# jialeli1/From-Voxel-to-Point

Measured on AMD Instinct MI355X. Metric: point clouds/sec fwd+bwd (FV2P, KITTI shape) at 1/2/4/8 MI355X, higher is better.
Workload: dtype f32

## Files before the change

### from-voxel-to-point_amd/fv2p_harness/fv2p_model.py

```python
import math
import os
from functools import partial

import numpy as np
import torch
import torch.nn as nn
import torch.nn.functional as F

from pcdet.ops.iou3d_nms import iou3d_nms_cuda, iou3d_nms_utils
from pcdet.ops.pointnet2.pointnet2_batch import pointnet2_modules as pn2_batch_modules
from pcdet.ops.pointnet2.pointnet2_batch import fused as pn2_fused
from pcdet.ops.pointnet2.pointnet2_batch import pointnet2_utils as pn2_batch
from pcdet.ops.pointnet2.pointnet2_stack import pointnet2_utils as pn2_stack
from pcdet.ops.roiaware_pool3d import roiaware_pool3d_utils
from pcdet.ops.roipoint_pool3d import roipoint_pool3d_utils
from pcdet.models.backbones_3d.pfe import bev_grid_pooling

import fv2p_native as _nat

from .backbone import VoxelResBackBone8x, bn_act

TWO_PI = 2.0 * math.pi


class FV2PConfig:
    point_cloud_range = (0.0, -40.0, -3.0, 70.4, 40.0, 1.0)
    voxel_size = (0.05, 0.05, 0.1)
    grid_size = (1408, 1600, 40)
    max_points_per_voxel, max_voxels = 5, 16000
    num_point_features = 4
    bev_layers, bev_strides, bev_filters = (5, 5), (1, 2), (128, 256)
    bev_up_strides, bev_up_filters = (1, 2), (256, 256)
    anchor_rotations = (0.0, 1.57)
    anchor_classes = (((3.9, 1.6, 1.56), -1.78, 0.6, 0.45), ((0.8, 0.6, 1.73), -0.6, 0.5, 0.35), ((1.76, 0.6, 1.73), -0.6, 0.5, 0.35))
    dir_offset, dir_limit_offset, num_dir_bins = 0.78539, 0.0, 2
    rpn_w = dict(cls=1.0, loc=2.0, dir=0.2)
    num_keypoints = 16384
    decode_levels = (("x_conv4", 8, 128, 256), ("x_conv3", 4, 64, 192), ("x_conv2", 2, 32, 160), ("x_conv1", 1, 16, 128))
    init_source, init_stride, init_channels = "x_conv4", 8, 128
    decoder_out = 128
    point_cls_fc, gt_extra_width, point_cls_weight = (64, 64), (0.2, 0.2, 0.2), 4.0
    nms_pre, nms_post, nms_thresh = 9000, 512, 0.8
    roi_per_image, fg_ratio = 128, 0.5
    cls_fg, cls_bg, cls_bg_lo, reg_fg, hard_bg_ratio = 0.75, 0.25, 0.1, 0.55, 0.8
    pool_extra_width, num_sampled_points, depth_normalizer = (3.2, 3.2, 3.2), 512, 70.0
    xyz_up, grid_size_roi = (128, 128), 6
    sa_radii, sa_nsamples, sa_mlps = (0.8, 1.6), (16, 32), ((64, 64), (64, 64))
    bev_pool_in, bev_pool_out = 512, 128
    interact_filters, cge_up, cge_interact, fuse_filters = (256, 256), (64, 64), (128,), (256,)
    cls_fc, reg_fc, dp_ratio = (256, 256), (256, 256), 0.3
    grad_norm_clip = 10.0
    key_stream = True
    point_branch_stream = True
    dense_branch_stream = False


class FV2PWaymoConfig(FV2PConfig):
    point_cloud_range = (-75.2, -75.2, -2.0, 75.2, 75.2, 4.0)
    voxel_size = (0.1, 0.1, 0.15)
    grid_size = (1504, 1504, 40)
    max_voxels = 80000
    num_point_features = 5
    bev_layers = (3, 3)
    anchor_classes = (((4.7, 2.1, 1.7), 0.0, 0.55, 0.4),)


KERNEL_GLUE = True
LINEAR_CHUNK_ROWS = 1024
FULL_NMS = False
_SIDE_STREAMS = {}
_CONSTS = {}
_CORNER_SIGNS = ((1, 1, -1), (1, -1, -1), (-1, -1, -1), (-1, 1, -1), (1, 1, 1), (1, -1, 1), (-1, -1, 1), (-1, 1, 1))


def dconst(like, values, dtype=torch.float32):
    key = (like.device, dtype, values)
    t = _CONSTS.get(key)
    if t is None:
        t = _CONSTS[key] = torch.tensor(values, dtype=dtype, device=like.device)
    return t


def side_stream(role, device):
    key = (role, torch.device(device).index)
    if key not in _SIDE_STREAMS:
        high = role in os.environ.get("FV2P_STREAM_PRIO", "dense").split(",")
        _SIDE_STREAMS[key] = torch.cuda.Stream(device=device, priority=-1 if high else 0)
    return _SIDE_STREAMS[key]


def limit_period(val, offset, period):
    return val - torch.floor(val / period + offset) * period


def rotate_z(points, angle):
    c, s = torch.cos(angle), torch.sin(angle)
    x, y = points[..., 0], points[..., 1]
    xr = x * c[:, None] - y * s[:, None]
    yr = x * s[:, None] + y * c[:, None]
# ... 2 lines not shown

def residual_encode(boxes, anchors):
    a_sz = anchors[..., 3:6].clamp_min(1e-5)
    b_sz = boxes[..., 3:6].clamp_min(1e-5)
    diag = torch.sqrt(a_sz[..., 0:1] ** 2 + a_sz[..., 1:2] ** 2)
    xy = (boxes[..., 0:2] - anchors[..., 0:2]) / diag
    z = (boxes[..., 2:3] - anchors[..., 2:3]) / a_sz[..., 2:3]
    return torch.cat((xy, z, torch.log(b_sz / a_sz), boxes[..., 6:7] - anchors[..., 6:7]), dim=-1)


def residual_decode(enc, anchors):
    a_sz = anchors[..., 3:6]
    diag = torch.sqrt(a_sz[..., 0:1] ** 2 + a_sz[..., 1:2] ** 2)
    xy = enc[..., 0:2] * diag + anchors[..., 0:2]
    z = enc[..., 2:3] * a_sz[..., 2:3] + anchors[..., 2:3]
    return torch.cat((xy, z, torch.exp(enc[..., 3:6]) * a_sz, enc[..., 6:7] + anchors[..., 6:7]), dim=-1)


def sigmoid_focal(logits, onehot, weights, alpha=0.25, gamma=2.0):
    p = torch.sigmoid(logits)
    alpha_w = onehot * alpha + (1 - onehot) * (1 - alpha)
    pt = onehot * (1.0 - p) + (1.0 - onehot) * p
    bce = logits.clamp(min=0) - logits * onehot + torch.log1p(torch.exp(-logits.abs()))
    return alpha_w * pt.pow(gamma) * bce * weights.unsqueeze(-1)


def smooth_l1(diff, beta):
    n = diff.abs()
    return torch.where(n < beta, 0.5 * n * n / beta, n - 0.5 * beta)


def box_corners(boxes):
    t = dconst(boxes, _CORNER_SIGNS, boxes.dtype) / 2
    c = boxes[:, None, 3:6] * t[None]
    return rotate_z(c, boxes[:, 6]) + boxes[:, None, 0:3]


def corner_loss_lidar(pred, gt):
    pc, gc = box_corners(pred), box_corners(gt)
    gflip = box_corners(torch.cat((gt[:, :6], gt[:, 6:7] + math.pi), dim=1))
    dist = torch.minimum((pc - gc).norm(dim=2), (pc - gflip).norm(dim=2))
    return smooth_l1(dist, 1.0).mean(dim=1)


def nearest_bev_boxes(b):
    rot = limit_period(b[..., 6], 0.5, math.pi).abs()
    swap = (rot >= math.pi / 4).unsqueeze(-1)
    dims = torch.where(swap, b[..., 3:5].flip(-1), b[..., 3:5])
    return torch.cat((b[..., 0:2] - dims / 2, b[..., 0:2] + dims / 2), dim=-1)


def mlp1d(cin, widths, out=None, conv=False, bn_kw=None, dropout_after_first=None):
    mk = (lambda a, b, bias: nn.Conv1d(a, b, 1, bias=bias)) if conv else (lambda a, b, bias: nn.Linear(a, b, bias=bias))
    layers = []
    for i, w in enumerate(widths):
        layers += [mk(cin, w, False), nn.BatchNorm1d(w, **(bn_kw or {})), nn.ReLU()]
        if dropout_after_first is not None and i == 0:
            layers.append(nn.Dropout(dropout_after_first))
        cin = w
    if out is not None:
        layers.append(mk(cin, out, True))
    return nn.Sequential(*layers)


def run_rows(seq, x):
    mods = list(seq)
    i = 0
    while i < len(mods):
        m = mods[i]
        if isinstance(m, nn.BatchNorm1d) and x.dim() == 2:
            relu = mods[i + 1] if i + 1 < len(mods) and isinstance(mods[i + 1], nn.ReLU) else None
            x = bn_act(m, x, relu)
            i += 1 + (relu is not None)
        elif (KERNEL_GLUE and type(m) is nn.Linear and x.dim() == 2 and x.is_cuda and x.shape[0] >= 4 * LINEAR_CHUNK_ROWS
              and x.shape[0] % LINEAR_CHUNK_ROWS == 0 and "forward" not in m.__dict__):
            x = rows_linear(x.reshape(-1, LINEAR_CHUNK_ROWS, x.shape[1]), m.weight, m.bias).reshape(x.shape[0], -1)
            i += 1
        else:
            x = m(x)
            i += 1
    return x


class BEVBackbone(nn.Module):

    def __init__(self, cfg, cin):
        super().__init__()
        bn = partial(nn.BatchNorm2d, eps=1e-3, momentum=0.01)
        self.blocks, self.deblocks = nn.ModuleList(), nn.ModuleList()
        for n, s, f, us, uf in zip(cfg.bev_layers, cfg.bev_strides, cfg.bev_filters, cfg.bev_up_strides, cfg.bev_up_filters):
            seq = [nn.ZeroPad2d(1), nn.Conv2d(cin, f, 3, stride=s, padding=0, bias=False), bn(f), nn.ReLU()]
            for _ in range(n):
                seq += [nn.Conv2d(f, f, 3, padding=1, bias=False), bn(f), nn.ReLU()]
            self.blocks.append(nn.Sequential(*seq))
            self.deblocks.append(nn.Sequential(nn.ConvTranspose2d(f, uf, us, stride=us, bias=False), bn(uf), nn.ReLU()))
            cin = f
        self.num_bev_features = sum(cfg.bev_up_filters)

    def forward(self, x):
        ups = []
        for blk, de in zip(self.blocks, self.deblocks):
            x = self._block(blk, x)
            ups.append(de(x))
        return torch.cat(ups, dim=1)

    @staticmethod
    def _block(blk, x):
        mods = list(blk)
        if (KERNEL_GLUE and len(mods) >= 2 and isinstance(mods[0], nn.ZeroPad2d) and type(mods[1]) is nn.Conv2d and "forward" not in mods[1].__dict__
                and tuple(mods[0].padding) == (1, 1, 1, 1) and tuple(mods[1].padding) == (0, 0) and mods[1].padding_mode == "zeros"):
            c = mods[1]
            x = F.conv2d(x, c.weight, c.bias, c.stride, (1, 1), c.dilation, c.groups)
            mods = mods[2:]
        for m in mods:
            x = m(x)
        return x


class AnchorLossFn(torch.autograd.Function):

    @staticmethod
    def forward(ctx, cls, box, dirs, labels, reg_t, anchor_rot, cfg):
        b, a = labels.shape
        out = cls.new_empty(4)
        dcls, dbox, ddirs = torch.empty_like(cls), torch.empty_like(box), torch.empty_like(dirs)
        with _nat.device_guard(cls.device):
            ws = _nat.workspace(int(_nat.lib().fv2p_anchor_loss_ws_bytes(b, a)), cls.device)
            _nat.call("fv2p_anchor_loss", cls, box, dirs, labels, reg_t, anchor_rot, b, a, 0.25, 1.0 / 9.0, float(cfg.dir_offset),
                      float(cfg.rpn_w["cls"]), float(cfg.rpn_w["loc"]), float(cfg.rpn_w["dir"]), out, dcls, dbox, ddirs, ws, ws.numel(), _nat.stream())
        ctx.save_for_backward(dcls, dbox, ddirs)
        return out[0]

    @staticmethod
    def backward(ctx, g):
        dcls, dbox, ddirs = ctx.saved_tensors
        return dcls * g, dbox * g, ddirs * g, None, None, None, None


class AnchorHead(nn.Module):

    def __init__(self, cfg, cin):
        super().__init__()
        self.cfg = cfg
        nr, nc = len(cfg.anchor_rotations), len(cfg.anchor_classes)
        na = nr * nc
        self.conv_cls = nn.Conv2d(cin, na, 1)
        self.conv_box = nn.Conv2d(cin, na * 7, 1)
        self.conv_dir_cls = nn.Conv2d(cin, na * cfg.num_dir_bins, 1)
        nn.init.constant_(self.conv_cls.bias, -math.log((1 - 0.01) / 0.01))
        nn.init.normal_(self.conv_box.weight, mean=0, std=0.001)
        r = cfg.point_cloud_range
        w, h = cfg.grid_size[0] // 8, cfg.grid_size[1] // 8
        xs = torch.arange(r[0], r[3] + 1e-5, step=(r[3] - r[0]) / (w - 1), dtype=torch.float32)
        ys = torch.arange(r[1], r[4] + 1e-5, step=(r[4] - r[1]) / (h - 1), dtype=torch.float32)
        a = torch.zeros(h, w, nc, nr, 7)
        a[..., 0] = xs.view(1, w, 1, 1)
        a[..., 1] = ys.view(h, 1, 1, 1)
        for c, (size, bottom, _, _) in enumerate(cfg.anchor_classes):
            a[:, :, c, :, 3:6] = torch.tensor(size)
            a[:, :, c, :, 2] = bottom
        a[..., 6] = torch.tensor(cfg.anchor_rotations).view(1, 1, 1, nr)
        a[..., 2] += a[..., 5] / 2
        self.register_buffer("anchors", a.view(-1, 7), persistent=False)
        self.register_buffer("anchor_rot", a.view(-1, 7)[:, 6].contiguous(), persistent=False)
        for c in range(nc):
            ac = a[:, :, c].reshape(-1, 7).contiguous()
            self.register_buffer(f"anchors_c{c}", ac, persistent=False)
            self.register_buffer(f"anchor_bev_c{c}", nearest_bev_boxes(ac), persistent=False)

    @torch.no_grad()
    def assign(self, gt):
        cfg = self.cfg
        nc, nr, b = len(cfg.anchor_classes), len(cfg.anchor_rotations), gt.shape[0]
        labels, regs = [], []
        for c, (_, _, matched, unmatched) in enumerate(cfg.anchor_classes):
            gt_c = gt if nc == 1 else torch.where((gt[..., 7:8] == c + 1), gt, torch.zeros_like(gt))
            one = self.assign_one_kernel if (gt.is_cuda and gt.shape[-1] >= 8 and KERNEL_GLUE) else self.assign_one_tensor_ops
            lab, reg = one(gt_c, getattr(self, f"anchors_c{c}"), getattr(self, f"anchor_bev_c{c}"), matched, unmatched)
            labels.append(lab.view(b, -1, 1, nr))
            regs.append(reg.view(b, -1, 1, nr, 7))
        if nc == 1:
            return labels[0].view(b, -1), regs[0].view(b, -1, 7)
        return torch.cat(labels, dim=2).reshape(b, -1), torch.cat(regs, dim=2).reshape(b, -1, 7)

    def assign_tensor_ops(self, gt):
        cfg = self.cfg
        nc, nr, b = len(cfg.anchor_classes), len(cfg.anchor_rotations), gt.shape[0]
        labels, regs = [], []
        for c, (_, _, matched, unmatched) in enumerate(cfg.anchor_classes):
            gt_c = gt if nc == 1 else torch.where((gt[..., 7:8] == c + 1), gt, torch.zeros_like(gt))
            lab, reg = self.assign_one_tensor_ops(gt_c, getattr(self, f"anchors_c{c}"), getattr(self, f"anchor_bev_c{c}"), matched, unmatched)
            labels.append(lab.view(b, -1, 1, nr))
            regs.append(reg.view(b, -1, 1, nr, 7))
        return torch.cat(labels, dim=2).reshape(b, -1), torch.cat(regs, dim=2).reshape(b, -1, 7)

    @staticmethod
    @torch.no_grad()
    def assign_one_kernel(gt, anchors, anchor_bev, matched, unmatched):
        b, g, a = gt.shape[0], gt.shape[1], anchors.shape[0]
# ... 574 lines not shown
```

### from-voxel-to-point_amd/fv2p_harness/mgaf_model.py

```python
from functools import partial

import math

import torch
import torch.nn as nn
import torch.nn.functional as F

from pcdet.ops.DeformableConvolutionV2PyTorch.modules.mdeformable_conv_block import MdeformConvBlock
from pcdet.ops.DeformableConvolutionV2PyTorch.modules.modulated_deform_conv import ModulatedDeformConv

from pcdet.ops.iou3d_nms import iou3d_nms_utils

from .backbone import VoxelResBackBone8x
from .fv2p_model import box_corners, sigmoid_focal


class MGAFConfig:
    grid_size = (1408, 1600, 40)
    num_point_features = 4
    layer_nums, layer_strides, num_filters = (5, 5, 5), (1, 2, 2), (128, 256, 256)
    upsample_strides, num_upsample_filters = (1, 2, 4), (256, 256, 256)
    shared_fc = (256,)
    head_deformable_groups = 4
    heads = (("hm", 3), ("offset", 2), ("height", 1), ("dim", 3), ("rot", 24), ("segm", 1), ("iouscore", 1))
    head_conv = 128
    point_cloud_range = (0.0, -40.0, -3.0, 70.4, 40.0, 1.0)
    voxel_size = (0.05, 0.05, 0.1)
    feature_map_stride, gaussian_minoverlap, gaussian_minradius, max_objs = 8, 0.01, 2, 50
    num_iouscore_training_samples = 24
    loss_weights = dict(hm=1.0, offset=1.0, height=1.0, dim=1.0, rot=1.0, segm=1.0, corner=1.0, iouscore=1.0)
    rot_bins, iou_fg_thresh, iou_bg_thresh = 12, 0.75, 0.25


class DCNBEVBackbone(nn.Module):
    def __init__(self, cfg, cin):
        super().__init__()
        bn = partial(nn.BatchNorm2d, eps=1e-3, momentum=0.01)
        self.blocks, self.deblocks = nn.ModuleList(), nn.ModuleList()
        for n, s, f, us, uf in zip(cfg.layer_nums, cfg.layer_strides, cfg.num_filters, cfg.upsample_strides, cfg.num_upsample_filters):
            seq = [nn.ZeroPad2d(1), nn.Conv2d(cin, f, 3, stride=s, padding=0, bias=False), bn(f), nn.ReLU()]
            for _ in range(n):
                seq += [nn.Conv2d(f, f, 3, padding=1, bias=False), bn(f), nn.ReLU()]
            self.blocks.append(nn.Sequential(*seq))
            self.deblocks.append(nn.Sequential(MdeformConvBlock(f, f, deformable_groups=1), bn(f), nn.ReLU(),
                                               nn.ConvTranspose2d(f, uf, us, stride=us, bias=False), bn(uf), nn.ReLU()))
            cin = f
        self.num_bev_features = sum(cfg.num_upsample_filters)

    def forward(self, x):
        ups = []
        from .fv2p_model import BEVBackbone
        for blk, de in zip(self.blocks, self.deblocks):
            x = BEVBackbone._block(blk, x)
            ups.append(de(x))
        return torch.cat(ups, dim=1)


class FeatureAdaption(nn.Module):

    def __init__(self, channels, deformable_groups):
        super().__init__()
        self.conv_offset_mask = nn.Conv2d(channels, deformable_groups * 27, 3, padding=1, bias=True)
        self.conv_adaption = ModulatedDeformConv(channels, channels, stride=1, kernel_size=3, padding=1, deformable_groups=deformable_groups, bias=False)

    def forward(self, x):
        o1, o2, mask = torch.chunk(self.conv_offset_mask(x), 3, dim=1)
        return torch.relu(self.conv_adaption(x, torch.cat((o1, o2), dim=1), torch.sigmoid(mask)))


class CenterAFHead(nn.Module):
    def __init__(self, cfg, cin):
        super().__init__()
        layers, pre = [], cin
        for f in cfg.shared_fc:
            layers += [nn.Conv2d(pre, f, 3, padding=1, bias=False), nn.BatchNorm2d(f), nn.ReLU()]
            pre = f
        self.shared_conv_layer = nn.Sequential(*layers)
        self.feature_adapt = FeatureAdaption(pre, cfg.head_deformable_groups)
        self.heads = nn.ModuleDict({name: nn.Sequential(nn.Conv2d(pre, cfg.head_conv, 3, padding=1, bias=False),
                                                        nn.BatchNorm2d(cfg.head_conv, eps=1e-3, momentum=0.01), nn.ReLU(),
                                                        nn.Conv2d(cfg.head_conv, out, 1, bias=True)) for name, out in cfg.heads})

    def forward(self, x):
        x = self.feature_adapt(self.shared_conv_layer(x))
        segm = self.heads["segm"](x)
        att = x + torch.sigmoid(segm.detach()).expand_as(x) * x
        preds = {"segm": segm}
        for name, head in self.heads.items():
            if name != "segm":
                preds[name] = head(att)
        return preds


def gaussian_radius(h, w, min_overlap):
    b1 = h + w
    c1 = w * h * (1 - min_overlap) / (1 + min_overlap)
    r1 = (b1 - torch.sqrt(b1 ** 2 - 4 * c1)) / 2
    b2 = 2 * (h + w)
    c2 = (1 - min_overlap) * w * h
    r2 = (b2 - torch.sqrt(b2 ** 2 - 16 * c2)) / 8
    a3 = 4 * min_overlap
    b3 = -2 * min_overlap * (h + w)
    c3 = (min_overlap - 1) * w * h
    r3 = (b3 + torch.sqrt(b3 ** 2 - 4 * a3 * c3)) / (2 * a3)
    return torch.minimum(torch.minimum(r1, r2), r3)


@torch.no_grad()
def center_targets(gt, cfg, num_classes):
    dev, b, m = gt.device, gt.shape[0], gt.shape[1]
    k = cfg.max_objs
    lo = torch.tensor(cfg.point_cloud_range[:3], dtype=torch.float32, device=dev)
    hi = torch.tensor(cfg.point_cloud_range[3:], dtype=torch.float32, device=dev)
    vs = torch.tensor(cfg.voxel_size, dtype=torch.float64, device=dev)
    stride = cfg.feature_map_stride
    sy = int(round((cfg.point_cloud_range[4] - cfg.point_cloud_range[1]) / cfg.voxel_size[1] / stride))
    sx = int(round((cfg.point_cloud_range[3] - cfg.point_cloud_range[0]) / cfg.voxel_size[0] / stride))
    boxes = gt[:, :, :7]
    nonzero = boxes.sum(-1) != 0
    pos = torch.arange(m, device=dev)
    last = torch.where(nonzero, pos, torch.zeros_like(pos)).amax(1)
    kk = min(k, m)
    bx = boxes[:, :kk]
    live = (pos[:kk][None] <= last[:, None])
    cls = gt[:, :kk, 7].to(torch.int8).long() - 1
    dimx = bx[..., 3].double() / vs[0] / stride
    dimy = bx[..., 4].double() / vs[1] / stride
    ok = live & (dimx > 0) & (dimy > 0)
    radius = gaussian_radius(torch.ceil(dimx), torch.ceil(dimy), cfg.gaussian_minoverlap)
    radius = torch.where(ok, radius, torch.zeros_like(radius)).nan_to_num(0.0).clamp(min=0).long().clamp(min=cfg.gaussian_minradius)
    cx = (bx[..., 0] - lo[0]).double() / vs[0] / stride
    cy = (bx[..., 1] - lo[1]).double() / vs[1] / stride
    cxi, cyi = torch.round(cx).long(), torch.round(cy).long()
    ok = ok & (cxi >= 0) & (cxi < sx) & (cyi >= 0) & (cyi < sy)
    ys = torch.arange(sy, device=dev).view(1, 1, sy, 1)
    xs = torch.arange(sx, device=dev).view(1, 1, 1, sx)
    dy, dx = ys - cyi[..., None, None], xs - cxi[..., None, None]
    r = radius[..., None, None]
# ... 171 lines not shown
```

### from-voxel-to-point_amd/pcdet/ops/spconv/norm.py

```python
import os

import torch
from torch import nn
from torch.autograd import Function

import fv2p_native as _nat

_ENABLED = os.environ.get("FV2P_FUSED_BN", "1") != "0"


_WS_BYTES = {}


def _ws_bytes(c):
    b = _WS_BYTES.get(c)
    if b is None:
        b = _WS_BYTES[c] = _nat.call("fv2p_batchnorm_ws_bytes", 0, c)
    return b


class _BatchNormReLU(Function):
    @staticmethod
    def forward(ctx, x, weight, bias, bn, relu):
        n, c = x.shape
        dev = x.device
        batch_stats = bn.training or bn.running_mean is None
        y = torch.empty_like(x)
        with _nat.device_guard(dev):
            if batch_stats:
                stats = torch.empty((2, c), dtype=torch.float32, device=dev)
                mean, invstd = stats[0], stats[1]
                track = bn.training and bn.running_mean is not None
                ws = _nat.workspace(_ws_bytes(c), dev)
                _nat.call("fv2p_batchnorm_forward", x, n, c, float(bn.eps), -1.0 if bn.momentum is None else float(bn.momentum),
                          weight, bias, int(relu), bn.running_mean if track else None, bn.running_var if track else None,
                          bn.num_batches_tracked if track else None, mean, invstd, y, ws, ws.numel(), _nat.stream())
            else:
                mean = bn.running_mean
                invstd = torch.rsqrt(bn.running_var + bn.eps)
                _nat.call("fv2p_batchnorm_apply", x, n, c, mean, invstd, weight, bias, int(relu), y, _nat.stream())
        ctx.save_for_backward(x, mean, invstd, weight, bias)
        ctx.relu, ctx.batch_stats = bool(relu), bool(batch_stats)
        return y

    @staticmethod
    def backward(ctx, dy):
        x, mean, invstd, weight, bias = ctx.saved_tensors
        n, c = x.shape
        dev = x.device
        dy = dy.contiguous()
        dx = torch.empty_like(x)
        dpar = torch.empty((2, c), dtype=torch.float32, device=dev)
        dgamma, dbeta = dpar[0], dpar[1]
        with _nat.device_guard(dev):
            ws = _nat.workspace(_ws_bytes(c), dev)
            _nat.call("fv2p_batchnorm_backward", x, dy, n, c, mean, invstd, weight, bias, int(ctx.relu), int(ctx.batch_stats),
                      dx, dgamma, dbeta, ws, ws.numel(), _nat.stream())
        return (dx if ctx.needs_input_grad[0] else None, dgamma if (weight is not None and ctx.needs_input_grad[1]) else None,
                dbeta if (bias is not None and ctx.needs_input_grad[2]) else None, None, None)


def _plain(module):
    return not (module._forward_hooks or module._forward_pre_hooks or module._backward_hooks)


def fusable(bn, relu_module, x, channels):
    if not _ENABLED or type(bn) is not nn.BatchNorm1d or not _plain(bn):
        return False
    if relu_module is not None and (type(relu_module) is not nn.ReLU or not _plain(relu_module)):
        return False
    if not (torch.is_tensor(x) and x.is_cuda and x.dtype == torch.float32 and x.dim() == 2):
        return False
    if torch.is_autocast_enabled() or channels != bn.num_features:
        return False
    c = channels
    if c > 256 and c % 4 != 0 or c > 1024:
        return False
    if bn.weight is not None and (bn.weight.dtype != torch.float32 or not bn.weight.is_cuda):
        return False
    return True


def batch_norm_relu(bn, x, relu_module=None):
    if not (torch.is_tensor(x) and x.dim() == 2 and x.is_contiguous() and fusable(bn, relu_module, x, x.shape[1])):
        return None
    if x.shape[0] < 2:
        return None
    ext = _nat.torch_ext()
    if ext is not None:
        return ext.batch_norm_relu(x, bn.weight, bn.bias, bn.running_mean, bn.running_var, bn.num_batches_tracked, bn.training,
                                   -1.0 if bn.momentum is None else float(bn.momentum), float(bn.eps), relu_module is not None)
    return _BatchNormReLU.apply(x, bn.weight, bn.bias, bn, relu_module is not None)
```

### include/fv2p_ops.h

```cpp
#ifndef FV2P_OPS_H_
#define FV2P_OPS_H_

#include <stddef.h>
#include <stdint.h>

#ifdef __cplusplus
extern "C" {
#endif

#define FV2P_ABI_VERSION 1

#define FV2P_EINVAL      (-1)
#define FV2P_EWORKSPACE  (-2)
#define FV2P_EHIP        (-3)
#define FV2P_ELIMIT      (-4)

typedef void* fv2p_stream_t;

const char* fv2p_last_error(void);
int fv2p_abi_version(void);

size_t fv2p_scan_ws_bytes(int64_t n);
int fv2p_exclusive_scan_i32(const int* in, int* out, int64_t n, int* total, void* ws, size_t ws_bytes,
                            fv2p_stream_t stream);
// ... 267 lines not shown
                      int deformable_group, float* dx_nhwc, float* doffset, float* dmask, float* dwt, void* ws,
                      size_t ws_bytes, fv2p_stream_t stream);
int fv2p_dcn_forward_grouped(const float* x_nhwc, const float* wt_oc, const float* bias, const float* offset,
                             const float* mask, int batch, int height, int width, int c_in, int c_out, int h_out,
                             int w_out, int kh, int kw, int sh, int sw, int ph, int pw, int dh, int dw,
                             int deformable_group, int group, float* y_nhwc, fv2p_stream_t stream);
size_t fv2p_dcn_backward_grouped_ws_bytes(int batch, int height, int width, int h_out, int w_out, int c_in, int c_out, int kh,
                                          int kw, int deformable_group, int group);
int fv2p_dcn_backward_grouped(const float* x_nhwc, const float* wt, const float* offset, const float* mask,
                              const float* dy_nhwc, int batch, int height, int width, int c_in, int c_out, int h_out,
                              int w_out, int kh, int kw, int sh, int sw, int ph, int pw, int dh, int dw,
                              int deformable_group, int group, float* dx_nhwc, float* doffset, float* dmask, float* dwt,
                              void* ws, size_t ws_bytes, fv2p_stream_t stream);

int fv2p_transpose_batched(const float* in, int batch, int64_t rows, int64_t cols, float* out, fv2p_stream_t stream);

int fv2p_deform_psroi_pool_forward(const float* data, const float* rois, const float* trans, int batch, int channels,
                                   int height, int width, int num_rois, int no_trans, float spatial_scale,
                                   int output_dim, int group_size, int pooled_size, int part_size,
                                   int sample_per_part, float trans_std, int num_classes, float* out,
                                   float* top_count, fv2p_stream_t stream);
int fv2p_deform_psroi_pool_backward(const float* grad_out, const float* data, const float* rois, const float* trans,
                                    const float* top_count, int batch, int channels, int height, int width,
                                    int num_rois, int no_trans, float spatial_scale, int output_dim,
                                    int group_size, int pooled_size, int part_size, int sample_per_part,
                                    float trans_std, int num_classes, float* grad_data, float* grad_trans,
                                    fv2p_stream_t stream);
size_t fv2p_deform_psroi_pool_backward_ws_bytes(int num_rois, int output_dim, int pooled_size, int sample_per_part);
int fv2p_deform_psroi_pool_backward_gather(const float* grad_out, const float* data, const float* rois, const float* trans,
                                           const float* top_count, int batch, int channels, int height, int width,
                                           int num_rois, int no_trans, float spatial_scale, int output_dim,
                                           int group_size, int pooled_size, int part_size, int sample_per_part,
                                           float trans_std, int num_classes, float* grad_data, float* grad_trans,
                                           void* ws, size_t ws_bytes, fv2p_stream_t stream);

size_t fv2p_batchnorm_ws_bytes(int64_t n, int c);
int fv2p_batchnorm_forward(const float* x, int64_t n, int c, float eps, float momentum, const float* gamma,
                           const float* beta, int relu, float* running_mean, float* running_var,
                           int64_t* num_batches_tracked, float* mean, float* invstd, float* y, void* ws,
                           size_t ws_bytes, fv2p_stream_t stream);
int fv2p_batchnorm_forward_stats(const float* x, int64_t n, int c, float eps, float momentum, const float* gamma,
                                 const float* beta, int relu, float* running_mean, float* running_var,
                                 int64_t* num_batches_tracked, float* mean, float* invstd, float* y,
                                 const double* stats, double* zero_next, int64_t zero_count, fv2p_stream_t stream);
int fv2p_batchnorm_backward_stats(const float* x, const float* dy, int64_t n, int c, const float* mean,
                                  const float* invstd, const float* gamma, const float* beta, int relu,
                                  int batch_stats, float* dx, float* dgamma, float* dbeta, const double* stats,
                                  double* zero_next, int64_t zero_count, fv2p_stream_t stream);
int fv2p_batchnorm_apply_res(const float* x, int64_t n, int c, const float* mean, const float* invstd, const float* gamma,
                             const float* beta, int relu, const float* residual, float* y, fv2p_stream_t stream);
int fv2p_batchnorm_backward_fin(const float* x, const float* dy, int64_t n, int c, const float* mean, const float* invstd,
                                const float* gamma, const float* beta, int relu, const float* coef, float* dx,
                                fv2p_stream_t stream);
int fv2p_batchnorm_backward_res(const float* x, const float* out, const float* dout, int64_t n, int c, const float* mean,
                                const float* invstd, const float* gamma, const float* beta, int batch_stats, float* dx,
                                float* dz, float* dgamma, float* dbeta, void* ws, size_t ws_bytes, fv2p_stream_t stream);
size_t fv2p_batchnorm_one_ws_bytes(int c);
int fv2p_batchnorm_one_pays(int64_t n, int c, int backward);
int fv2p_batchnorm_forward_one(const float* x, int64_t n, int c, float eps, float momentum, const float* gamma, const float* beta,
                               int relu, float* running_mean, float* running_var, int64_t* num_batches_tracked, float* mean,
                               float* invstd, const float* residual, float* y, void* ws, size_t ws_bytes, unsigned* counters,
                               fv2p_stream_t stream);
int fv2p_batchnorm_backward_one(const float* x, const float* dy, int64_t n, int c, const float* mean, const float* invstd,
                                const float* gamma, const float* beta, int relu, int batch_stats, const float* mask_y, float* dx,
                                float* dz_out, float* dgamma, float* dbeta, void* ws, size_t ws_bytes, unsigned* counters,
                                fv2p_stream_t stream);
size_t fv2p_batchnorm_wide_ws_bytes(int c);
int fv2p_batchnorm_wide_counter_words(int c);
int fv2p_batchnorm_forward_wide(const float* x, int64_t n, int c, float eps, float momentum, const float* gamma, const float* beta,
                                int relu, float* running_mean, float* running_var, int64_t* num_batches_tracked, float* mean,
                                float* invstd, const float* residual, float* y, void* ws, size_t ws_bytes, unsigned* counters,
                                fv2p_stream_t stream);
int fv2p_batchnorm_backward_wide(const float* x, const float* dy, int64_t n, int c, const float* mean, const float* invstd,
                                 const float* gamma, const float* beta, int relu, int batch_stats, const float* mask_y, float* dx,
                                 float* dz_out, float* dgamma, float* dbeta, void* ws, size_t ws_bytes, unsigned* counters,
                                 fv2p_stream_t stream);
int fv2p_batchnorm_apply(const float* x, int64_t n, int c, const float* mean, const float* invstd,
                         const float* gamma, const float* beta, int relu, float* y, fv2p_stream_t stream);
int fv2p_batchnorm_backward(const float* x, const float* dy, int64_t n, int c, const float* mean,
                            const float* invstd, const float* gamma, const float* beta, int relu, int batch_stats,
                            float* dx, float* dgamma, float* dbeta, void* ws, size_t ws_bytes,
                            fv2p_stream_t stream);

#ifdef __cplusplus
}
#endif
#endif
```

Baseline: 104.5.

## Fuse BatchNorm2d+ReLU in BEV backbone and write deblock outputs into concat buffer

```diff
diff --git a/from-voxel-to-point_amd/csrc/batchnorm2d.hip b/from-voxel-to-point_amd/csrc/batchnorm2d.hip
--- /dev/null
+++ b/from-voxel-to-point_amd/csrc/batchnorm2d.hip
@@ -0,0 +1,328 @@
+#include "common.hpp"
+#include "bn_fold.hpp"
+
+namespace fv2p {
+
+struct Bn2dGeom {
+  int b, c, k;
+  long long plane;
+  long long chunk;
+};
+
+constexpr long long kBn2dChunk = 8192;
+constexpr int kBn2dMaxChunks = 64;
+constexpr int kBn2dSerialFold = 32;
+
+static void bn2d_geom(int b, int c, long long plane, Bn2dGeom* g) {
+  long long k = (plane + kBn2dChunk / 2) / kBn2dChunk;
+  if (k < 1) k = 1;
+  if (k > kBn2dMaxChunks) k = kBn2dMaxChunks;
+  long long chunk = ceil_div(ceil_div(plane, k), 4) * 4;
+  k = ceil_div(plane, chunk);
+  g->b = b; g->c = c; g->k = static_cast<int>(k); g->plane = plane; g->chunk = chunk;
+}
+
+__device__ __forceinline__ void bn2d_block(const Bn2dGeom& g, int* b, int* c, int* k) {
+  const unsigned id = blockIdx.x;
+  *k = static_cast<int>(id % g.k);
+  const unsigned pl = id / g.k;
+  *c = static_cast<int>(pl % g.c);
+  *b = static_cast<int>(pl / g.c);
+}
+
+__device__ __forceinline__ void bn2d_block_sum(double& a, double& b, double (*red)[4]) {
+#pragma unroll
+  for (int off = 32; off >= 1; off >>= 1) {
+    a += __shfl_down(a, off, 64);
+    b += __shfl_down(b, off, 64);
+  }
+  const int tid = threadIdx.x;
+  if ((tid & 63) == 0) { red[0][tid >> 6] = a; red[1][tid >> 6] = b; }
+  __syncthreads();
+  if (tid == 0) {
+    a = ((red[0][0] + red[0][1]) + red[0][2]) + red[0][3];
+    b = ((red[1][0] + red[1][1]) + red[1][2]) + red[1][3];
+  }
+}
+
+__device__ __forceinline__ void bn2d_fold(const double* __restrict__ p, int count, double (*red)[256], double* a_out, double* b_out) {
+  double a = 0.0, b = 0.0;
+  if (count <= kBn2dSerialFold) {
+    for (int q = 0; q < count; ++q) { a += p[2 * q]; b += p[2 * q + 1]; }
+  } else {
+    const int tid = threadIdx.x;
+    for (int q = tid; q < count; q += 256) { a += p[2 * q]; b += p[2 * q + 1]; }
+    red[0][tid] = a; red[1][tid] = b;
+    __syncthreads();
+    for (int s = 128; s >= 1; s >>= 1) {
+      if (tid < s) { red[0][tid] += red[0][tid + s]; red[1][tid] += red[1][tid + s]; }
+      __syncthreads();
+    }
+    a = red[0][0]; b = red[1][0];
+  }
+  *a_out = a; *b_out = b;
+}
+
+template <int V>
+struct Vec2d;
+template <>
+struct Vec2d<4> {
+  float v[4];
+  __device__ __forceinline__ void load(const float* p) { const float4 q = *reinterpret_cast<const float4*>(p); v[0] = q.x; v[1] = q.y; v[2] = q.z; v[3] = q.w; }
+  __device__ __forceinline__ void store(float* p) const { *reinterpret_cast<float4*>(p) = make_float4(v[0], v[1], v[2], v[3]); }
+};
+template <>
+struct Vec2d<1> {
+  float v[1];
+  __device__ __forceinline__ void load(const float* p) { v[0] = *p; }
+  __device__ __forceinline__ void store(float* p) const { *p = v[0]; }
+};
+
+template <int V, bool BWD>
+__global__ __launch_bounds__(256) void bn2d_reduce_k(const float* __restrict__ x, const float* __restrict__ dy, long long dy_bstride, int dy_coff,
+                                                     Bn2dGeom g, const float* __restrict__ mean, const float* __restrict__ invstd,
+                                                     const float* __restrict__ gamma, const float* __restrict__ beta, int relu,
+                                                     double* __restrict__ partial, long long* __restrict__ nbt, long long* __restrict__ nbt_copy) {
+  __shared__ double red[2][4];
+  int b, c, k;
+  bn2d_block(g, &b, &c, &k);
+  const int tid = threadIdx.x;
+  if (!BWD && nbt && blockIdx.x == 0 && tid == 0) {
+    const long long seen = *nbt;
+    *nbt_copy = seen;
+    *nbt = seen + 1;
+  }
+  const long long e0 = static_cast<long long>(k) * g.chunk;
+  const long long e1 = min(e0 + g.chunk, g.plane);
+  const float* xp = x + (static_cast<long long>(b) * g.c + c) * g.plane;
+  const float* gp = BWD ? dy + static_cast<long long>(b) * dy_bstride + static_cast<long long>(dy_coff + c) * g.plane : nullptr;
+  float m = 0.f, is = 0.f, ga = 1.f, be = 0.f;
+  if (BWD) { m = mean[c]; is = invstd[c]; ga = gamma ? gamma[c] : 1.f; be = beta ? beta[c] : 0.f; }
+  double s1 = 0.0, s2 = 0.0;
+  auto accumulate = [&](const Vec2d<V>& xv, const Vec2d<V>& gv) {
+#pragma unroll
+    for (int i = 0; i < V; ++i) {
+      if (!BWD) {
+        const double d = xv.v[i];
+        s1 += d; s2 += d * d;
+      } else {
+        const float xhat = (xv.v[i] - m) * is;
+        const float t = xhat * ga + be;
+        const float dz = (relu && !(t > 0.f)) ? 0.f : gv.v[i];
+        s1 += dz; s2 += static_cast<double>(dz) * xhat;
+      }
+    }
+  };
+  constexpr int U = 4;
+  constexpr long long step = 256 * V;
+  long long e = e0 + static_cast<long long>(tid) * V;
+  for (; e + (U - 1) * step < e1; e += U * step) {
+    Vec2d<V> xv[U], gv[U];
+#pragma unroll
+    for (int u = 0; u < U; ++u) {
+      xv[u].load(xp + e + u * step);
+      if (BWD) gv[u].load(gp + e + u * step);
+    }
+#pragma unroll
+    for (int u = 0; u < U; ++u) accumulate(xv[u], gv[u]);
+  }
+  for (; e < e1; e += step) {
+    Vec2d<V> xv, gv;
+    xv.load(xp + e);
+    if (BWD) gv.load(gp + e);
+    accumulate(xv, gv);
+  }
+  bn2d_block_sum(s1, s2, red);
+  if (tid == 0) {
+    double* p = partial + ((static_cast<long long>(c) * g.b + b) * g.k + k) * 2;
+    p[0] = s1; p[1] = s2;
+  }
+}
+
+template <int V>
+__global__ __launch_bounds__(256) void bn2d_apply_fwd_k(const float* __restrict__ x, Bn2dGeom g, const double* __restrict__ partial, BnFwdFin ff,
+                                                        const float* __restrict__ gamma, const float* __restrict__ beta, int relu,
+                                                        float* __restrict__ y, long long y_bstride, int y_coff) {
+  __shared__ double red[2][256];
+  __shared__ float sh[2];
+  int b, c, k;
+  bn2d_block(g, &b, &c, &k);
+  const int tid = threadIdx.x;
+  const int count = g.b * g.k;
+  double sa, sb;
+  bn2d_fold(partial + static_cast<long long>(c) * count * 2, count, red, &sa, &sb);
+  if (tid == 0) {
+    float mu_f, is_f;
+    bn_fwd_channel(sa, sb, static_cast<long long>(g.b) * g.plane, ff, c, b == 0 && k == 0, &mu_f, &is_f);
+    sh[0] = mu_f; sh[1] = is_f;
+  }
+  __syncthreads();
+  const float m = sh[0], is = sh[1];
+  const float ga = gamma ? gamma[c] : 1.f, be = beta ? beta[c] : 0.f;
+  const long long e0 = static_cast<long long>(k) * g.chunk;
+  const long long e1 = min(e0 + g.chunk, g.plane);
+  const float* xp = x + (static_cast<long long>(b) * g.c + c) * g.plane;
+  float* yp = y + static_cast<long long>(b) * y_bstride + static_cast<long long>(y_coff + c) * g.plane;
+  auto apply = [&](const Vec2d<V>& xv, Vec2d<V>& o) {
+#pragma unroll
+    for (int i = 0; i < V; ++i) {
+      const float xhat = (xv.v[i] - m) * is;
+      const float t = xhat * ga + be;
+      o.v[i] = (relu && t <= 0.f) ? 0.f : t;
+    }
+  };
+  constexpr int U = 4;
+  constexpr long long step = 256 * V;
+  long long e = e0 + static_cast<long long>(tid) * V;
+  for (; e + (U - 1) * step < e1; e += U * step) {
+    Vec2d<V> xv[U], o[U];
+#pragma unroll
+    for (int u = 0; u < U; ++u) xv[u].load(xp + e + u * step);
+#pragma unroll
+    for (int u = 0; u < U; ++u) { apply(xv[u], o[u]); o[u].store(yp + e + u * step); }
+  }
+  for (; e < e1; e += step) {
+    Vec2d<V> xv, o;
+    xv.load(xp + e);
+    apply(xv, o);
+    o.store(yp + e);
+  }
+}
+
+template <int V>
+__global__ __launch_bounds__(256) void bn2d_apply_bwd_k(const float* __restrict__ x, const float* __restrict__ dy, long long dy_bstride, int dy_coff,
+                                                        Bn2dGeom g, const double* __restrict__ partial, const float* __restrict__ mean,
+                                                        const float* __restrict__ invstd, const float* __restrict__ gamma,
+                                                        const float* __restrict__ beta, int relu, float* __restrict__ dx,
+                                                        float* __restrict__ dgamma, float* __restrict__ dbeta) {
+  __shared__ double red[2][256];
+  int b, c, k;
+  bn2d_block(g, &b, &c, &k);
+  const int tid = threadIdx.x;
+  const int count = g.b * g.k;
+  double sa, sb;
+  bn2d_fold(partial + static_cast<long long>(c) * count * 2, count, red, &sa, &sb);
+  if (tid == 0 && b == 0 && k == 0) {
+    dbeta[c] = static_cast<float>(sa);
+    dgamma[c] = static_cast<float>(sb);
+  }
+  const double n = static_cast<double>(g.b) * static_cast<double>(g.plane);
+  const float c1 = static_cast<float>(sa / n), c2 = static_cast<float>(sb / n);
+  const float m = mean[c], is = invstd[c];
+  const float ga = gamma ? gamma[c] : 1.f, be = beta ? beta[c] : 0.f;
+  const long long e0 = static_cast<long long>(k) * g.chunk;
+  const long long e1 = min(e0 + g.chunk, g.plane);
+  const long long xoff = (static_cast<long long>(b) * g.c + c) * g.plane;
+  const float* xp = x + xoff;
+  float* dxp = dx + xoff;
+  const float* gp = dy + static_cast<long long>(b) * dy_bstride + static_cast<long long>(dy_coff + c) * g.plane;
+  auto apply = [&](const Vec2d<V>& xv, const Vec2d<V>& gv, Vec2d<V>& o) {
+#pragma unroll
+    for (int i = 0; i < V; ++i) {
+      const float xhat = (xv.v[i] - m) * is;
+      const float t = xhat * ga + be;
+      const float dz = (relu && !(t > 0.f)) ? 0.f : gv.v[i];
+      o.v[i] = ga * is * (dz - c1 - xhat * c2);
+    }
+  };
+  constexpr int U = 4;
+  constexpr long long step = 256 * V;
+  long long e = e0 + static_cast<long long>(tid) * V;
+  for (; e + (U - 1) * step < e1; e += U * step) {
+    Vec2d<V> xv[U], gv[U], o[U];
+#pragma unroll
+    for (int u = 0; u < U; ++u) { xv[u].load(xp + e + u * step); gv[u].load(gp + e + u * step); }
+#pragma unroll
+    for (int u = 0; u < U; ++u) { apply(xv[u], gv[u], o[u]); o[u].store(dxp + e + u * step); }
+  }
+  for (; e < e1; e += step) {
+    Vec2d<V> xv, gv, o;
+    xv.load(xp + e);
+    gv.load(gp + e);
+    apply(xv, gv, o);
+    o.store(dxp + e);
+  }
+}
+
+static bool bn2d_aligned16(const void* p) { return (reinterpret_cast<uintptr_t>(p) & 15) == 0; }
+
+static int bn2d_check(const char* who, int b, int c, int64_t plane, int64_t bstride, int coff) {
+  FV2P_REQUIRE(b >= 1 && c >= 1 && plane >= 1, FV2P_EINVAL, "%s: b=%d c=%d plane=%lld", who, b, c, static_cast<long long>(plane));
+  FV2P_REQUIRE(static_cast<long long>(b) * plane >= 2, FV2P_EINVAL, "%s: one value per channel", who);
+  FV2P_REQUIRE(coff >= 0 && bstride >= static_cast<int64_t>(coff + c) * plane, FV2P_EINVAL, "%s: channels %d..%d do not fit a batch stride of %lld", who,
+               coff, coff + c, static_cast<long long>(bstride));
+  return 0;
+}
+
+}
+
+using namespace fv2p;
+
+extern "C" size_t fv2p_batchnorm2d_ws_bytes(int b, int c, int64_t plane) {
+  Bn2dGeom g;
+  bn2d_geom(b > 0 ? b : 1, c > 0 ? c : 1, plane > 0 ? plane : 1, &g);
+  Sizer s;
+  s.take<double>(static_cast<size_t>(g.c) * g.b * g.k * 2);
+  s.take<long long>(1);
+  return s.bytes();
+}
+
+extern "C" int fv2p_batchnorm2d_forward(const float* x, int b, int c, int64_t plane, float eps, float momentum, const float* gamma,
+                                        const float* beta, int relu, float* running_mean, float* running_var, int64_t* num_batches_tracked,
+                                        float* mean, float* invstd, float* y, int64_t y_batch_stride, int y_channel_offset, void* ws,
+                                        size_t ws_bytes, fv2p_stream_t stream_) {
+  hipStream_t stream = static_cast<hipStream_t>(stream_);
+  if (int rc = bn2d_check("batchnorm2d_forward", b, c, plane, y_batch_stride, y_channel_offset)) return rc;
+  FV2P_REQUIRE(x && y && mean && invstd && ws, FV2P_EINVAL, "batchnorm2d_forward: null pointer");
+  FV2P_REQUIRE((running_mean == nullptr) == (running_var == nullptr), FV2P_EINVAL, "batchnorm2d_forward: running_mean and running_var come together");
+  FV2P_REQUIRE(ws_bytes >= fv2p_batchnorm2d_ws_bytes(b, c, plane), FV2P_EWORKSPACE, "batchnorm2d_forward: workspace %lld < %lld",
+               static_cast<long long>(ws_bytes), static_cast<long long>(fv2p_batchnorm2d_ws_bytes(b, c, plane)));
+  Bn2dGeom g;
+  bn2d_geom(b, c, plane, &g);
+  const int64_t blocks = static_cast<int64_t>(b) * c * g.k;
+  FV2P_REQUIRE(blocks <= 0x7fffffff, FV2P_ELIMIT, "batchnorm2d_forward: %lld workgroups", static_cast<long long>(blocks));
+  Carver cv(ws, ws_bytes);
+  double* partial = cv.take<double>(static_cast<size_t>(g.c) * g.b * g.k * 2);
+  long long* nbt_copy = cv.take<long long>(1);
+  long long* nbt = (running_mean && num_batches_tracked) ? reinterpret_cast<long long*>(num_batches_tracked) : nullptr;
+  BnFwdFin ff{mean, invstd, running_mean, running_var, nbt ? nbt_copy : nullptr, momentum, eps};
+  const bool vec = (plane % 4 == 0) && bn2d_aligned16(x) && bn2d_aligned16(y) && (y_batch_stride % 4 == 0);
+  const dim3 grid(static_cast<unsigned>(blocks)), wg(256);
+  if (vec) {
+    hipLaunchKernelGGL((bn2d_reduce_k<4, false>), grid, wg, 0, stream, x, nullptr, 0ll, 0, g, nullptr, nullptr, nullptr, nullptr, 0, partial, nbt, nbt_copy);
+    hipLaunchKernelGGL((bn2d_apply_fwd_k<4>), grid, wg, 0, stream, x, g, partial, ff, gamma, beta, relu, y, static_cast<long long>(y_batch_stride), y_channel_offset);
+  } else {
+    hipLaunchKernelGGL((bn2d_reduce_k<1, false>), grid, wg, 0, stream, x, nullptr, 0ll, 0, g, nullptr, nullptr, nullptr, nullptr, 0, partial, nbt, nbt_copy);
+    hipLaunchKernelGGL((bn2d_apply_fwd_k<1>), grid, wg, 0, stream, x, g, partial, ff, gamma, beta, relu, y, static_cast<long long>(y_batch_stride), y_channel_offset);
+  }
+  FV2P_LAUNCH_CHECK();
+  return 0;
+}
+
+extern "C" int fv2p_batchnorm2d_backward(const float* x, const float* dy, int64_t dy_batch_stride, int dy_channel_offset, int b, int c,
+                                         int64_t plane, const float* mean, const float* invstd, const float* gamma, const float* beta,
+                                         int relu, float* dx, float* dgamma, float* dbeta, void* ws, size_t ws_bytes, fv2p_stream_t stream_) {
+  hipStream_t stream = static_cast<hipStream_t>(stream_);
+  if (int rc = bn2d_check("batchnorm2d_backward", b, c, plane, dy_batch_stride, dy_channel_offset)) return rc;
+  FV2P_REQUIRE(x && dy && mean && invstd && dx && dgamma && dbeta && ws, FV2P_EINVAL, "batchnorm2d_backward: null pointer");
+  FV2P_REQUIRE(ws_bytes >= fv2p_batchnorm2d_ws_bytes(b, c, plane), FV2P_EWORKSPACE, "batchnorm2d_backward: workspace %lld < %lld",
+               static_cast<long long>(ws_bytes), static_cast<long long>(fv2p_batchnorm2d_ws_bytes(b, c, plane)));
+  Bn2dGeom g;
+  bn2d_geom(b, c, plane, &g);
+  const int64_t blocks = static_cast<int64_t>(b) * c * g.k;
+  FV2P_REQUIRE(blocks <= 0x7fffffff, FV2P_ELIMIT, "batchnorm2d_backward: %lld workgroups", static_cast<long long>(blocks));
+  Carver cv(ws, ws_bytes);
+  double* partial = cv.take<double>(static_cast<size_t>(g.c) * g.b * g.k * 2);
+  const bool vec = (plane % 4 == 0) && bn2d_aligned16(x) && bn2d_aligned16(dy) && bn2d_aligned16(dx) && (dy_batch_stride % 4 == 0);
+  const dim3 grid(static_cast<unsigned>(blocks)), wg(256);
+  const long long gs = static_cast<long long>(dy_batch_stride);
+  if (vec) {
+    hipLaunchKernelGGL((bn2d_reduce_k<4, true>), grid, wg, 0, stream, x, dy, gs, dy_channel_offset, g, mean, invstd, gamma, beta, relu, partial, nullptr, nullptr);
+    hipLaunchKernelGGL((bn2d_apply_bwd_k<4>), grid, wg, 0, stream, x, dy, gs, dy_channel_offset, g, partial, mean, invstd, gamma, beta, relu, dx, dgamma, dbeta);
+  } else {
+    hipLaunchKernelGGL((bn2d_reduce_k<1, true>), grid, wg, 0, stream, x, dy, gs, dy_channel_offset, g, mean, invstd, gamma, beta, relu, partial, nullptr, nullptr);
+    hipLaunchKernelGGL((bn2d_apply_bwd_k<1>), grid, wg, 0, stream, x, dy, gs, dy_channel_offset, g, partial, mean, invstd, gamma, beta, relu, dx, dgamma, dbeta);
+  }
+  FV2P_LAUNCH_CHECK();
+  return 0;
+}
diff --git a/from-voxel-to-point_amd/fv2p_harness/fv2p_model.py b/from-voxel-to-point_amd/fv2p_harness/fv2p_model.py
--- a/from-voxel-to-point_amd/fv2p_harness/fv2p_model.py
+++ b/from-voxel-to-point_amd/fv2p_harness/fv2p_model.py
@@ -15,6 +15,7 @@
 from pcdet.ops.roiaware_pool3d import roiaware_pool3d_utils
 from pcdet.ops.roipoint_pool3d import roipoint_pool3d_utils
 from pcdet.models.backbones_3d.pfe import bev_grid_pooling
+from pcdet.ops.spconv.norm import batch_norm_relu_2d, batch_norm_relu_2d_cat
 
 import fv2p_native as _nat
 
@@ -183,6 +184,39 @@
     return x
 
 
+def dense_seq(mods, x):
+    i = 0
+    while i < len(mods):
+        m = mods[i]
+        if KERNEL_GLUE and type(m) is nn.BatchNorm2d:
+            relu = mods[i + 1] if i + 1 < len(mods) and type(mods[i + 1]) is nn.ReLU else None
+            y = batch_norm_relu_2d(m, x, relu)
+            if y is not None:
+                x = y
+                i += 1 + (relu is not None)
+                continue
+        x = m(x)
+        i += 1
+    return x
+
+
+def deblock_head(de, x):
+    mods = list(de)
+    if (KERNEL_GLUE and len(mods) >= 3 and type(mods[-2]) is nn.BatchNorm2d and type(mods[-1]) is nn.ReLU
+            and not (de._forward_hooks or de._forward_pre_hooks or de._backward_hooks)):
+        return mods[-2], dense_seq(mods[:-2], x), mods[-1]
+    return de(x)
+
+
+def cat_deblocks(ups):
+    if len(ups) > 1 and all(isinstance(u, tuple) for u in ups):
+        y = batch_norm_relu_2d_cat(ups)
+        if y is not None:
+            return y
+    ups = [dense_seq([u[0], u[2]], u[1]) if isinstance(u, tuple) else u for u in ups]
+    return torch.cat(ups, dim=1) if len(ups) > 1 else ups[0]
+
+
 class BEVBackbone(nn.Module):
 
     def __init__(self, cfg, cin):
@@ -202,8 +236,8 @@
         ups = []
         for blk, de in zip(self.blocks, self.deblocks):
             x = self._block(blk, x)
-            ups.append(de(x))
-        return torch.cat(ups, dim=1)
+            ups.append(deblock_head(de, x))
+        return cat_deblocks(ups)
 
     @staticmethod
     def _block(blk, x):
@@ -213,9 +247,7 @@
             c = mods[1]
             x = F.conv2d(x, c.weight, c.bias, c.stride, (1, 1), c.dilation, c.groups)
             mods = mods[2:]
-        for m in mods:
-            x = m(x)
-        return x
+        return dense_seq(mods, x)
 
 
 class AnchorLossFn(torch.autograd.Function):
diff --git a/from-voxel-to-point_amd/fv2p_harness/mgaf_model.py b/from-voxel-to-point_amd/fv2p_harness/mgaf_model.py
--- a/from-voxel-to-point_amd/fv2p_harness/mgaf_model.py
+++ b/from-voxel-to-point_amd/fv2p_harness/mgaf_model.py
@@ -49,11 +49,11 @@
 
     def forward(self, x):
         ups = []
-        from .fv2p_model import BEVBackbone
+        from .fv2p_model import BEVBackbone, cat_deblocks, deblock_head
         for blk, de in zip(self.blocks, self.deblocks):
             x = BEVBackbone._block(blk, x)
-            ups.append(de(x))
-        return torch.cat(ups, dim=1)
+            ups.append(deblock_head(de, x))
+        return cat_deblocks(ups)
 
 
 class FeatureAdaption(nn.Module):
diff --git a/from-voxel-to-point_amd/pcdet/ops/spconv/norm.py b/from-voxel-to-point_amd/pcdet/ops/spconv/norm.py
--- a/from-voxel-to-point_amd/pcdet/ops/spconv/norm.py
+++ b/from-voxel-to-point_amd/pcdet/ops/spconv/norm.py
@@ -91,3 +91,127 @@
         return ext.batch_norm_relu(x, bn.weight, bn.bias, bn.running_mean, bn.running_var, bn.num_batches_tracked, bn.training,
                                    -1.0 if bn.momentum is None else float(bn.momentum), float(bn.eps), relu_module is not None)
     return _BatchNormReLU.apply(x, bn.weight, bn.bias, bn, relu_module is not None)
+
+
+_WS_BYTES_2D = {}
+
+
+def _ws_bytes_2d(b, c, plane):
+    key = (b, c, plane)
+    n = _WS_BYTES_2D.get(key)
+    if n is None:
+        n = _WS_BYTES_2D[key] = _nat.call("fv2p_batchnorm2d_ws_bytes", b, c, plane)
+    return n
+
+
+def _bn2d_forward(bn, x, weight, bias, relu, out, c_off):
+    b, c = x.shape[0], x.shape[1]
+    plane = x.shape[2] * x.shape[3]
+    stats = torch.empty((2, c), dtype=torch.float32, device=x.device)
+    track = bn.running_mean is not None
+    ws = _nat.workspace(_ws_bytes_2d(b, c, plane), x.device)
+    _nat.call("fv2p_batchnorm2d_forward", x, b, c, plane, float(bn.eps), -1.0 if bn.momentum is None else float(bn.momentum), weight, bias,
+              int(relu), bn.running_mean if track else None, bn.running_var if track else None, bn.num_batches_tracked if track else None,
+              stats[0], stats[1], out, out.shape[1] * plane, c_off, ws, ws.numel(), _nat.stream())
+    return stats[0], stats[1]
+
+
+def _bn2d_backward(x, dy, c_off, mean, invstd, weight, bias, relu):
+    b, c = x.shape[0], x.shape[1]
+    plane = x.shape[2] * x.shape[3]
+    dx = torch.empty_like(x)
+    dpar = torch.empty((2, c), dtype=torch.float32, device=x.device)
+    ws = _nat.workspace(_ws_bytes_2d(b, c, plane), x.device)
+    _nat.call("fv2p_batchnorm2d_backward", x, dy, dy.shape[1] * plane, c_off, b, c, plane, mean, invstd, weight, bias, int(relu), dx, dpar[0], dpar[1],
+              ws, ws.numel(), _nat.stream())
+    return dx, dpar[0], dpar[1]
+
+
+class _BatchNormReLU2d(Function):
+    @staticmethod
+    def forward(ctx, x, weight, bias, bn, relu):
+        y = torch.empty_like(x)
+        with _nat.device_guard(x.device):
+            mean, invstd = _bn2d_forward(bn, x, weight, bias, relu, y, 0)
+        ctx.save_for_backward(x, mean, invstd, weight, bias)
+        ctx.relu = bool(relu)
+        return y
+
+    @staticmethod
+    def backward(ctx, dy):
+        x, mean, invstd, weight, bias = ctx.saved_tensors
+        with _nat.device_guard(x.device):
+            dx, dgamma, dbeta = _bn2d_backward(x, dy.contiguous(), 0, mean, invstd, weight, bias, ctx.relu)
+        return (dx if ctx.needs_input_grad[0] else None, dgamma if (weight is not None and ctx.needs_input_grad[1]) else None,
+                dbeta if (bias is not None and ctx.needs_input_grad[2]) else None, None, None)
+
+
+class _BatchNormReLU2dCat(Function):
+
+    @staticmethod
+    def forward(ctx, bns, relus, *tensors):
+        xs = tensors[0::3]
+        b, h, w = xs[0].shape[0], xs[0].shape[2], xs[0].shape[3]
+        out = xs[0].new_empty((b, sum(x.shape[1] for x in xs), h, w))
+        saved, c_off = [], 0
+        with _nat.device_guard(out.device):
+            for i, x in enumerate(xs):
+                weight, bias = tensors[3 * i + 1], tensors[3 * i + 2]
+                mean, invstd = _bn2d_forward(bns[i], x, weight, bias, relus[i], out, c_off)
+                saved += [x, mean, invstd, weight, bias]
+                c_off += x.shape[1]
+        ctx.save_for_backward(*saved)
+        ctx.relus = tuple(bool(r) for r in relus)
+        return out
+
+    @staticmethod
+    def backward(ctx, dy):
+        saved = ctx.saved_tensors
+        dy = dy.contiguous()
+        grads, c_off = [None, None], 0
+        with _nat.device_guard(dy.device):
+            for i in range(len(saved) // 5):
+                x, mean, invstd, weight, bias = saved[5 * i:5 * i + 5]
+                need = ctx.needs_input_grad[2 + 3 * i:5 + 3 * i]
+                if any(need):
+                    dx, dgamma, dbeta = _bn2d_backward(x, dy, c_off, mean, invstd, weight, bias, ctx.relus[i])
+                    grads += [dx if need[0] else None, dgamma if (weight is not None and need[1]) else None,
+                              dbeta if (bias is not None and need[2]) else None]
+                else:
+                    grads += [None, None, None]
+                c_off += x.shape[1]
+        return tuple(grads)
+
+
+def fusable_2d(bn, relu_module, x):
+    if not _ENABLED or type(bn) is not nn.BatchNorm2d or not _plain(bn) or not bn.training:
+        return False
+    if relu_module is not None and (type(relu_module) is not nn.ReLU or not _plain(relu_module)):
+        return False
+    if not (torch.is_tensor(x) and x.is_cuda and x.dtype == torch.float32 and x.dim() == 4 and x.is_contiguous()):
+        return False
+    if torch.is_autocast_enabled() or x.shape[1] != bn.num_features or x.shape[0] * x.shape[2] * x.shape[3] < 2:
+        return False
+    for p in (bn.weight, bn.bias, bn.running_mean, bn.running_var):
+        if p is not None and (p.dtype != torch.float32 or p.device != x.device):
+            return False
+    return True
+
+
+def batch_norm_relu_2d(bn, x, relu_module=None):
+    if not fusable_2d(bn, relu_module, x):
+        return None
+    return _BatchNormReLU2d.apply(x, bn.weight, bn.bias, bn, relu_module is not None)
+
+
+def batch_norm_relu_2d_cat(layers):
+    if not layers:
+        return None
+    x0 = layers[0][1]
+    for bn, x, relu_module in layers:
+        if not fusable_2d(bn, relu_module, x) or x.device != x0.device or x.shape[0] != x0.shape[0] or x.shape[2:] != x0.shape[2:]:
+            return None
+    args = []
+    for bn, x, _ in layers:
+        args += [x, bn.weight, bn.bias]
+    return _BatchNormReLU2dCat.apply([bn for bn, _, _ in layers], [relu_module is not None for _, _, relu_module in layers], *args)
diff --git a/include/fv2p_ops.h b/include/fv2p_ops.h
--- a/include/fv2p_ops.h
+++ b/include/fv2p_ops.h
@@ -373,6 +373,16 @@
                             float* dx, float* dgamma, float* dbeta, void* ws, size_t ws_bytes,
                             fv2p_stream_t stream);
 
+size_t fv2p_batchnorm2d_ws_bytes(int b, int c, int64_t plane);
+int fv2p_batchnorm2d_forward(const float* x, int b, int c, int64_t plane, float eps, float momentum, const float* gamma,
+                             const float* beta, int relu, float* running_mean, float* running_var,
+                             int64_t* num_batches_tracked, float* mean, float* invstd, float* y, int64_t y_batch_stride,
+                             int y_channel_offset, void* ws, size_t ws_bytes, fv2p_stream_t stream);
+int fv2p_batchnorm2d_backward(const float* x, const float* dy, int64_t dy_batch_stride, int dy_channel_offset, int b, int c,
+                              int64_t plane, const float* mean, const float* invstd, const float* gamma, const float* beta,
+                              int relu, float* dx, float* dgamma, float* dbeta, void* ws, size_t ws_bytes,
+                              fv2p_stream_t stream);
+
 #ifdef __cplusplus
 }
 #endif
```

Measured after the change: 107.2, median of 5. 2.6% higher.
